# ruivieira/ccfd-demo-summit

Measured on AMD Instinct MI355X. Metric: transactions/sec (whole node) + p50 scoring latency at 1/2/4/8 MI355X, higher is better.
Workload: dtype bf16

## Files before the change

### csrc/kernels/g32_core.h

```cpp
#pragma once

#include <cstdlib>
#include <cstring>

#include <type_traits>

#include "common.h"
#include "rules.h"

#ifndef CCFD_G32_TREE_BLOCK
#define CCFD_G32_TREE_BLOCK 4
#endif

namespace ccfd {

constexpr int kG32Rows = 64;
constexpr int kG32Waves = 4;
constexpr int kG32LeafLds = 16384;
constexpr int kG32Tb = CCFD_G32_TREE_BLOCK;

struct G32Row { uint4 lo, hi; };

__device__ __forceinline__ void g32_fetch(const unsigned char* __restrict__ x, int n, int chunk, int lane,
                                          G32Row& r) {
  const long last = (long)n * CCFD_G32_ROW_BYTES - 16;
  const long b0 = (long)chunk * (kG32Rows * CCFD_G32_ROW_BYTES) + 16 * lane;
  r.lo = ld_g16(x + min(b0, last));
  r.hi = ld_g16(x + min(b0 + 1024, last));
}

__device__ __forceinline__ void g32_rows(uint4* __restrict__ t, int lane, G32Row& r) {
  t[lane] = r.lo;
  t[64 + lane] = r.hi;
  __builtin_amdgcn_wave_barrier();
  __builtin_amdgcn_fence(__ATOMIC_SEQ_CST, "wavefront");
  r.lo = t[2 * lane];
  r.hi = t[2 * lane + 1];
  __builtin_amdgcn_wave_barrier();
  __builtin_amdgcn_fence(__ATOMIC_SEQ_CST, "wavefront");
}

__device__ __forceinline__ unsigned g32_byte(const G32Row& r, int j) {
  const unsigned w = j < 4 ? r.lo.x : j < 8 ? r.lo.y : j < 12 ? r.lo.z : j < 16 ? r.lo.w
                   : j < 20 ? r.hi.x : j < 24 ? r.hi.y : j < 28 ? r.hi.z : r.hi.w;
  return (w >> (8 * (j & 3))) & 0xffu;
}

constexpr int kG20Words = CCFD_G20_ROW_BYTES / 4;

__device__ __forceinline__ void g20_fetch(const unsigned char* __restrict__ x, int n, int chunk, int lane,
                                          G32Row& r) {
  const unsigned* __restrict__ xw = reinterpret_cast<const unsigned*>(x);
  const long last = (long)n * kG20Words - 1;
  const long w0 = (long)chunk * (kG32Rows * kG20Words) + lane;
  r.lo.x = ld_g(xw + min(w0, last));
  r.lo.y = ld_g(xw + min(w0 + 64, last));
  r.lo.z = ld_g(xw + min(w0 + 128, last));
  r.lo.w = ld_g(xw + min(w0 + 192, last));
  r.hi.x = ld_g(xw + min(w0 + 256, last));
}

__device__ __forceinline__ void g20_rows(uint4* __restrict__ t4, int lane, G32Row& r) {
  unsigned* t = reinterpret_cast<unsigned*>(t4);
  t[lane] = r.lo.x;
  t[64 + lane] = r.lo.y;
  t[128 + lane] = r.lo.z;
  t[192 + lane] = r.lo.w;
  t[256 + lane] = r.hi.x;
  __builtin_amdgcn_wave_barrier();
  __builtin_amdgcn_fence(__ATOMIC_SEQ_CST, "wavefront");
  const unsigned* q = t + kG20Words * lane;
  r.lo.x = q[0];
  r.lo.y = q[1];
  r.lo.z = q[2];
  r.lo.w = q[3];
  r.hi.x = q[4];
  __builtin_amdgcn_wave_barrier();
  __builtin_amdgcn_fence(__ATOMIC_SEQ_CST, "wavefront");
}

__device__ __forceinline__ unsigned g20_lift(const G32Row& r, unsigned (&b)[kF]) {
  const unsigned w[kG20Words + 1] = {r.lo.x, r.lo.y, r.lo.z, r.lo.w, r.hi.x, 0u};
#pragma unroll
  for (int j = 0; j < kF; ++j) {
    const int bit = 5 * j, wi = bit >> 5, sh = bit & 31;
    b[j] = (sh + 5 <= 32 ? (w[wi] >> sh) : __builtin_amdgcn_alignbit(w[wi + 1], w[wi], sh)) & 31u;
  }
  return ((r.hi.x >> 22) & 0xfu) | ((r.hi.x >> 26) << 8);
}

typedef const __attribute__((address_space(4))) int* g32_cint_p;

template <int D, int R>
__device__ __forceinline__ void g32_trees(const unsigned (&b0)[kF], const unsigned (&b1)[kF],
                                          const float* __restrict__ lv, g32_cint_p feat, g32_cint_p kbin, int T,
                                          float (&acc)[R]) {
  constexpr int L = 1 << D;
#pragma unroll
  for (int q = 0; q < R; ++q) acc[q] = 0.f;
  auto tree = [&](int t, const int* fs, const int* ks) __attribute__((always_inline)) {
    unsigned i0 = 0, i1 = 0;
#pragma unroll
    for (int d = D - 1; d >= 0; --d) {
      const int f = fs[d];
      const unsigned k = (unsigned)ks[d];
      i0 = __builtin_amdgcn_alignbit(i0, k - b0[f], 31);
      if constexpr (R == 2) i1 = __builtin_amdgcn_alignbit(i1, k - b1[f], 31);
    }
    acc[0] += lv[t * L + (int)i0];
    if constexpr (R == 2) acc[R - 1] += lv[t * L + (int)i1];
  };
  int t = 0;
  for (; t + kG32Tb <= T; t += kG32Tb) {
    int fb[kG32Tb * D], kb[kG32Tb * D];
#pragma unroll
    for (int j = 0; j < kG32Tb * D; ++j) { fb[j] = feat[t * D + j]; kb[j] = kbin[t * D + j]; }
#pragma unroll
    for (int k = 0; k < kG32Tb; ++k) tree(t + k, fb + k * D, kb + k * D);
  }
  for (; t < T; ++t) {
    int fb[D], kb[D];
#pragma unroll
    for (int j = 0; j < D; ++j) { fb[j] = feat[t * D + j]; kb[j] = kbin[t * D + j]; }
    tree(t, fb, kb);
  }
}

__device__ __forceinline__ unsigned g32_lift(const G32Row& r, unsigned (&b)[kF]) {
#pragma unroll
  for (int j = 0; j < kF; ++j) b[j] = g32_byte(r, j);
  return r.hi.w >> 16;
}

template <bool kG20>
__device__ __forceinline__ void gx_fetch(const unsigned char* __restrict__ x, int n, int chunk, int lane, G32Row& r) {
  if constexpr (kG20) g20_fetch(x, n, chunk, lane, r);
  else g32_fetch(x, n, chunk, lane, r);
}
template <bool kG20>
__device__ __forceinline__ void gx_rows(uint4* __restrict__ t, int lane, G32Row& r) {
  if constexpr (kG20) g20_rows(t, lane, r);
  else g32_rows(t, lane, r);
}
template <bool kG20>
__device__ __forceinline__ unsigned gx_lift(const G32Row& r, unsigned (&b)[kF]) {
  if constexpr (kG20) return g20_lift(r, b);
  else return g32_lift(r, b);
}

struct G32Model {
  g32_cint_p feat, kbin;
  const float* leaves;
  float base;
  unsigned stamp;
};

template <int D>
__device__ __forceinline__ G32Model g32_model(const void* blob_, int T) {
  const char* blob = reinterpret_cast<const char*>(blob_);
  return G32Model{(g32_cint_p)gbb_section(blob, T, D, 0), (g32_cint_p)gbb_section(blob, T, D, 1),
                  reinterpret_cast<const float*>(gbb_section(blob, T, D, 2)), gbb_base(blob),
                  (unsigned)*reinterpret_cast<const int*>(blob + 20)};
}

template <int D>
__device__ __forceinline__ void g32_stage_leaves(const float* src, int T, float* lv, int tid, int nthreads) {
  constexpr int L = 1 << D;
  const float4* s4 = reinterpret_cast<const float4*>(src);
  float4* d4 = reinterpret_cast<float4*>(lv);
  const int nl = T * L;
  for (int i = tid; i < nl / 4; i += nthreads) d4[i] = s4[i];
  for (int i = (nl & ~3) + tid; i < nl; i += nthreads) lv[i] = src[i];
}

template <int D, bool kGL>
__device__ __forceinline__ const float* g32_leaves(const G32Model& M, int T, float* lv, int tid, int nthreads) {
  if constexpr (kGL) return M.leaves;
  g32_stage_leaves<D>(M.leaves, T, lv, tid, nthreads);
  return lv;
}

struct G32Wave {
  unsigned fraud = 0, rows = 0, stale = 0;
  unsigned long long psum = 0;
};

struct G32RowOut {
  bool valid, fresh, fr;
  float p;
  unsigned long long m;
};

template <bool kR, bool kProba = false>
__device__ __forceinline__ G32RowOut g32_row_epilogue(EpilogueLds& epi, G32Wave& w, const G32Model& M, unsigned meta,
                                                      float acc, int row, int n, float threshold,
                                                      const ccfd_rule_prog* rules, float* proba, uint8_t* route) {
  const bool valid = row < n;
  const bool fresh = ((meta >> 8) & 0xffu) == M.stamp;
  float p_fresh;
  if constexpr (kProba) p_fresh = acc;
  else p_fresh = sigmoid(M.base + acc);
  const float p = fresh ? p_fresh : __builtin_nanf("");
  bool fr;
  if constexpr (kR) fr = valid && fresh && rule_route(rules, p, [](int) { return 0.f; });
  else fr = valid && fresh && (p >= threshold);
  if (valid) {
#ifndef CCFD_EXP_NO_OUTPUTS
    if (proba) st_g(proba + row, p);
    if (route) st_g(route + row, (uint8_t)(fr ? 1 : 0));
#endif
    if (fresh) w.psum += (unsigned)(p * 1e6f + 0.5f);
    if (fresh) atomicAdd(&epi.hist[(fr ? kNB : 0) + min((int)(meta & 0xffu), kNB - 1)], 1u);
  }
  const unsigned long long m = __ballot(fr);
  w.fraud += __popcll(m);
  w.rows += __popcll(__ballot(valid));
  w.stale += __popcll(__ballot(valid && !fresh));
  return G32RowOut{valid, fresh, fr, p, m};
}

__device__ __forceinline__ void g32_wave_commit(EpilogueLds& epi, G32Wave& w, unsigned long long* cnt, int lane) {
  w.psum = wave_sum_u64(w.psum);
  if (lane == 0) {
    atomicAdd(&epi.fraud, w.fraud);
    atomicAdd(&epi.rows, w.rows);
    atomicAdd(&epi.psum_e6, w.psum);
  }
  if (cnt != nullptr && lane == 0 && w.stale) atomicAdd(&cnt[CCFD_CNT_WIRE_STALE], (unsigned long long)w.stale);
}

__device__ __forceinline__ void g32_item_commit(EpilogueLds& epi, G32Wave& w, unsigned long long* cnt, int lane) {
  w.psum = wave_sum_u64(w.psum);
  if (lane == 0 && w.rows) {
    atomicAdd(&epi.fraud, w.fraud);
    atomicAdd(&epi.rows, w.rows);
    atomicAdd(&epi.psum_e6, w.psum);
    if (w.stale && cnt) atomicAdd(&cnt[CCFD_CNT_WIRE_STALE], (unsigned long long)w.stale);
  }
  w = G32Wave{};
}

inline int g32_env(const char* name, int dflt, int lo, int hi) {
  const char* e = getenv(name);
  if (!e) return dflt;
  const int v = atoi(e);
  return v < lo || v > hi ? dflt : v;
}

}
```

Measured before the change: 892.2 million.

## Software-pipeline tree-walk scalar loads and LDS leaf reads in g32_trees

Restructures the tree-ensemble inner loop into a double-buffered pipeline. Scalar loads of feature and threshold indices for group g+2 are issued while group g is walked. Leaf reads are deferred and summed one step later, separated by explicit lgkmcnt waits and sched_barriers. Group size is now derived from tree depth. The aim is to hide scalar-load and LDS latency behind ALU work, at the cost of more registers and a hard-coded waitcnt encoding that may be wrong for the target ISA.

```diff
diff --git a/csrc/kernels/g32_core.h b/csrc/kernels/g32_core.h
--- a/csrc/kernels/g32_core.h
+++ b/csrc/kernels/g32_core.h
@@ -91,38 +91,94 @@
 
 typedef const __attribute__((address_space(4))) int* g32_cint_p;
 
+constexpr int g32_group(int D, int R) {
+  const int g = 12 / D < 2 ? 2 : (12 / D > kG32Tb ? kG32Tb : 12 / D);
+  return R == 2 ? 2 : g;
+}
+static_assert(kG32Tb >= 2, "CCFD_G32_TREE_BLOCK: at least two trees");
+
+constexpr int kWaitLgkm0 = 0xC07F;
+
 template <int D, int R>
 __device__ __forceinline__ void g32_trees(const unsigned (&b0)[kF], const unsigned (&b1)[kF],
                                           const float* __restrict__ lv, g32_cint_p feat, g32_cint_p kbin, int T,
                                           float (&acc)[R]) {
   constexpr int L = 1 << D;
+  constexpr int G = g32_group(D, R);
+  constexpr int P = G * D;
 #pragma unroll
   for (int q = 0; q < R; ++q) acc[q] = 0.f;
-  auto tree = [&](int t, const int* fs, const int* ks) __attribute__((always_inline)) {
-    unsigned i0 = 0, i1 = 0;
+  auto walk = [&](const int* fs, const int* ks, unsigned (&ix)[R]) __attribute__((always_inline)) {
+#pragma unroll
+    for (int q = 0; q < R; ++q) ix[q] = 0;
 #pragma unroll
     for (int d = D - 1; d >= 0; --d) {
       const int f = fs[d];
       const unsigned k = (unsigned)ks[d];
-      i0 = __builtin_amdgcn_alignbit(i0, k - b0[f], 31);
-      if constexpr (R == 2) i1 = __builtin_amdgcn_alignbit(i1, k - b1[f], 31);
+      ix[0] = __builtin_amdgcn_alignbit(ix[0], k - b0[f], 31);
+      if constexpr (R == 2) ix[R - 1] = __builtin_amdgcn_alignbit(ix[R - 1], k - b1[f], 31);
     }
-    acc[0] += lv[t * L + (int)i0];
-    if constexpr (R == 2) acc[R - 1] += lv[t * L + (int)i1];
   };
-  int t = 0;
-  for (; t + kG32Tb <= T; t += kG32Tb) {
-    int fb[kG32Tb * D], kb[kG32Tb * D];
-#pragma unroll
-    for (int j = 0; j < kG32Tb * D; ++j) { fb[j] = feat[t * D + j]; kb[j] = kbin[t * D + j]; }
-#pragma unroll
-    for (int k = 0; k < kG32Tb; ++k) tree(t + k, fb + k * D, kb + k * D);
-  }
-  for (; t < T; ++t) {
-    int fb[D], kb[D];
-#pragma unroll
-    for (int j = 0; j < D; ++j) { fb[j] = feat[t * D + j]; kb[j] = kbin[t * D + j]; }
-    tree(t, fb, kb);
+  auto leaf = [&](int t, unsigned i) __attribute__((always_inline)) {
+    const unsigned off = ((unsigned)(t * L) + i) * 4u;
+    return *reinterpret_cast<const float*>(reinterpret_cast<const char*>(lv) + off);
+  };
+  const int NG = T / G;
+  if (NG > 0) {
+    int fa[P], ka[P], fb[P], kb[P];
+    float pend[G * R];
+#pragma unroll
+    for (int j = 0; j < G * R; ++j) pend[j] = 0.f;
+    typedef const __attribute__((address_space(4))) char* cchar_p;
+    auto load = [&](int g, int (&f)[P], int (&k)[P]) __attribute__((always_inline)) {
+      const unsigned off = (unsigned)(g * P) * 4u;
+      const g32_cint_p fg = (g32_cint_p)((cchar_p)feat + off), kg = (g32_cint_p)((cchar_p)kbin + off);
+#pragma unroll
+      for (int j = 0; j < P; ++j) { f[j] = fg[j]; k[j] = kg[j]; }
+    };
+    auto step = [&](int g, int (&f)[P], int (&k)[P]) __attribute__((always_inline)) {
+      unsigned ix[G][R];
+#pragma unroll
+      for (int j = 0; j < G; ++j) walk(f + j * D, k + j * D, ix[j]);
+      __builtin_amdgcn_sched_barrier(0);
+      __builtin_amdgcn_s_waitcnt(kWaitLgkm0);
+      __builtin_amdgcn_sched_barrier(0);
+#pragma unroll
+      for (int j = 0; j < G; ++j) {
+#pragma unroll
+        for (int q = 0; q < R; ++q) acc[q] += pend[j * R + q];
+      }
+#pragma unroll
+      for (int j = 0; j < G; ++j) {
+#pragma unroll
+        for (int q = 0; q < R; ++q) pend[j * R + q] = leaf(g * G + j, ix[j][q]);
+      }
+      load(min(g + 2, NG - 1), f, k);
+      __builtin_amdgcn_sched_barrier(0);
+    };
+    load(0, fa, ka);
+    load(min(1, NG - 1), fb, kb);
+    __builtin_amdgcn_s_waitcnt(kWaitLgkm0);
+    int g = 0;
+    for (; g + 1 < NG; g += 2) {
+      step(g, fa, ka);
+      step(g + 1, fb, kb);
+    }
+    if (g < NG) step(g, fa, ka);
+#pragma unroll
+    for (int j = 0; j < G; ++j) {
+#pragma unroll
+      for (int q = 0; q < R; ++q) acc[q] += pend[j * R + q];
+    }
+  }
+  for (int t = NG * G; t < T; ++t) {
+    int f1[D], k1[D];
+#pragma unroll
+    for (int j = 0; j < D; ++j) { f1[j] = feat[t * D + j]; k1[j] = kbin[t * D + j]; }
+    unsigned ix[R];
+    walk(f1, k1, ix);
+#pragma unroll
+    for (int q = 0; q < R; ++q) acc[q] += leaf(t, ix[q]);
   }
 }
 
```

Result: no change. 892.7 million, median of 3 (+0.1%).
